# fuxiao0719/PanopticNeRF

Measured on AMD Instinct MI355X. Metric: Msamples/sec (coarse+fine), KITTI-360 1408x376, higher is better.
Workload: dtype bf16

## Files before the change

include/pnr.h:

```cpp
#ifndef PNR_H
#define PNR_H
#include <stdint.h>

#ifdef __cplusplus
extern "C" {
#endif

#define PNR_OK 0
#define PNR_EINVAL (-1)
#define PNR_EHIP (-2)
#define PNR_ENODEV (-3)

#define PNR_PREC_BF16 0
#define PNR_PREC_FP32 1

int pnr_version(void);
const char* pnr_last_error(void);
int pnr_device_check(int dev, char* buf_host, int buflen);

int pnr_stratified(const float* rays, int64_t n_rays, int n_samples, int lindisp,
                   const float* t_rand, float* z_out, void* stream);

int pnr_points(const float* rays, const float* z, int64_t n_rays, int n_samples, float* pts_out,
               void* stream);
// ... 3 lines not shown
typedef struct pnr_mlp_desc {
    int32_t D, W, skip;
    int32_t xyz_L, dir_L;
    int32_t n_sem, n_inst, head_W;
    int32_t precision;
    int32_t plan;
    int32_t head_tap;
    int32_t head_depth;
    int32_t schedule;
    int32_t clk_probe[2];
    int32_t flags;
} pnr_mlp_desc;

#define PNR_MLP_SOFTMAX 1
#define PNR_MLP_WG_CAP(n) (((n) & 0x1FF) << 16)
#define PNR_MLP_TRACE 0x7A00

typedef struct pnr_mlp_params_host {
    const float* const* pts_w; const float* const* pts_b;
    const float* alpha_w; const float* alpha_b;
    const float* feature_w; const float* feature_b;
    const float* views_w; const float* views_b;
    const float* rgb_w; const float* rgb_b;
    const float* sem0_w; const float* sem0_b; const float* sem1_w; const float* sem1_b;
    const float* inst0_w; const float* inst0_b; const float* inst1_w; const float* inst1_b;
} pnr_mlp_params_host;

int64_t pnr_mlp_packed_bytes(const pnr_mlp_desc* desc);
int pnr_mlp_pack(const pnr_mlp_desc* desc, const pnr_mlp_params_host* params, void* packed_host);

// ... 7 lines not shown
                    int64_t n_rays, int n_samples, float* raw, int64_t raw_stride_s,
                    int64_t raw_stride_c, void* stream);

int pnr_mlp_fused_plan(const pnr_mlp_desc* desc);
int64_t pnr_mlp_forward_composite_workspace_bytes(const pnr_mlp_desc* desc, int64_t n_rays, int n_samples, int want_weights);
int pnr_mlp_forward_composite(const pnr_mlp_desc* desc, const void* packed, const float* rays, const float* z,
                              int64_t n_rays, int n_samples, const int32_t* label_sem, const int32_t* label_inst,
                              int white_bkgd, float* rgb, float* depth, float* acc, float* weights, float* sem,
                              float* inst, float* fix_sem, float* fix_inst, void* workspace, void* stream);

int pnr_mlp_forward_tiles(const pnr_mlp_desc* desc, const void* packed, const float* rays, const float* z, int64_t n_rays,
                          int n_samples, void* workspace, void* stream);
int pnr_composite_combine(const pnr_mlp_desc* desc, const void* workspace, const float* z, int64_t n_rays, int n_samples,
                          const int32_t* label_sem, const int32_t* label_inst, int white_bkgd, float* rgb, float* depth,
                          float* acc, float* weights, float* sem, float* inst, float* fix_sem, float* fix_inst, void* stream);

int pnr_mlp_query(const pnr_mlp_desc* desc, const void* packed, const float* points, int64_t n_points,
                  float* sigma, int32_t* sem_label, int32_t* inst_label, int32_t* panoptic, const int32_t* is_thing,
                  float* sem_logits, float* inst_logits, int64_t logit_stride, void* stream);
int pnr_mlp_query_supported(const pnr_mlp_desc* desc);

int pnr_mlp_train_layout(const pnr_mlp_desc* desc, int64_t n_samples, int64_t* acts_off_host ,
                         int64_t* dys_off_host );
int pnr_mlp_forward_train(const pnr_mlp_desc* desc, const void* packed, const float* rays, const float* z,
                          int64_t n_rays, int n_samples, float* raw, int64_t raw_stride_s,
                          int64_t raw_stride_c, void* acts, void* stream);
int64_t pnr_mlp_bwd_packed_bytes(const pnr_mlp_desc* desc);
int pnr_mlp_pack_bwd(const pnr_mlp_desc* desc, const pnr_mlp_params_host* params, void* packed_host);
int pnr_mlp_backward(const pnr_mlp_desc* desc, const void* packed_bwd, const float* d_raw, const void* acts,
                     void* dys, int64_t n_rays, int n_samples, void* stream);
// ... 144 lines not shown
```

panopticnerf_amd/_lib.py:

```python
import ctypes
import os

_HERE = os.path.dirname(os.path.abspath(__file__))
LIB_PATH = os.environ.get("PNR_LIB_PATH") or os.path.join(_HERE, "libpnr.so")

c_f = ctypes.c_void_p
c_i64 = ctypes.c_int64
c_int = ctypes.c_int

PREC_BF16, PREC_FP32 = 0, 1
MLP_SOFTMAX, MLP_TRACE = 1, 0x7A00
CAMERA_PINHOLE, CAMERA_FISHEYE = 0, 1
TAG_PIXEL, TAG_FRAME = 16, 17
SAMPLE_POOLED, SAMPLE_FRAME = 0, 1


class LossCfg(ctypes.Structure):
    _fields_ = [("w_rgb", ctypes.c_float), ("w_depth", ctypes.c_float), ("w_sem", ctypes.c_float),
                ("w_fix_sem", ctypes.c_float), ("w_inst", ctypes.c_float), ("w_fix_inst", ctypes.c_float),
                ("depth_l2", ctypes.c_int32), ("fix_eps", ctypes.c_float), ("maps_are_prob", ctypes.c_int32)]


class MlpDesc(ctypes.Structure):
    _fields_ = [("D", ctypes.c_int32), ("W", ctypes.c_int32), ("skip", ctypes.c_int32),
                ("xyz_L", ctypes.c_int32), ("dir_L", ctypes.c_int32),
                ("n_sem", ctypes.c_int32), ("n_inst", ctypes.c_int32), ("head_W", ctypes.c_int32),
# ... 69 lines not shown
    "pnr_gen_rays": (c_int, [ctypes.POINTER(ctypes.c_float), ctypes.POINTER(ctypes.c_float), c_int, c_int, ctypes.c_float,
                             ctypes.c_float, c_f, c_i64, c_f, c_f]),
    "pnr_gen_rays_fisheye": (c_int, [ctypes.POINTER(ctypes.c_float), ctypes.POINTER(ctypes.c_float), c_int, c_int, ctypes.c_float,
                                     ctypes.c_float, c_f, c_i64, c_f, c_f, c_f]),
    "pnr_project_points": (c_int, [c_int, ctypes.POINTER(ctypes.c_float), ctypes.POINTER(ctypes.c_float), c_int, c_int, c_f, c_i64,
                                   c_f, c_f, c_f, c_f]),
    "pnr_panoptic_labels": (c_int, [c_f, c_f, c_f, c_i64, c_int, c_int, c_f, c_f, c_f, c_f]),
    "pnr_confusion": (c_int, [c_f, c_f, c_i64, c_int, c_f, c_f]),
    "pnr_sample_pdf": (c_int, [c_f, c_f, c_f, c_i64, c_int, c_int, c_f, c_f, c_f, c_f]),
    "pnr_bbox_hits": (c_int, [c_f, c_i64, c_f, c_int, c_int, c_f, c_f, c_f, c_f]),
    "pnr_restrict_rays": (c_int, [c_f, c_i64, c_f, c_f, c_int, c_f, c_f]),
    "pnr_sample_labels": (c_int, [c_f, c_i64, c_int, c_f, c_f, c_f, c_int, c_f, c_f, c_f, c_f]),
    "pnr_ray_setup": (c_int, [c_f, c_i64, c_f, c_int, c_int, c_f, c_int, c_int, c_f, c_int, c_f, c_f, c_f, c_f, c_f, c_f, c_f]),
    "pnr_sample_pdf_labels": (c_int, [c_f, c_f, c_f, c_i64, c_int, c_int, c_f, c_f, c_f, c_f, c_int, c_f, c_f, c_f, c_f]),
    "pnr_mlp_forward_tiles": (c_int, [ctypes.POINTER(MlpDesc), c_f, c_f, c_f, c_i64, c_int, c_f, c_f]),
    "pnr_rng_begin": (c_int, [c_f, c_f, c_f]),
    "pnr_rng_fill": (c_int, [ctypes.POINTER(RngDesc), c_i64, c_int, c_int, c_f, c_f]),
    "pnr_stratified_rng": (c_int, [c_f, c_i64, c_int, c_int, ctypes.POINTER(RngDesc), c_f, c_f]),
    "pnr_ray_setup_rng": (c_int, [c_f, c_i64, c_f, c_int, c_int, c_f, c_int, c_int, ctypes.POINTER(RngDesc), c_int, c_f, c_f, c_f, c_f,
                                  c_f, c_f, c_f]),
    "pnr_sample_pdf_rng": (c_int, [c_f, c_f, ctypes.POINTER(RngDesc), c_i64, c_int, c_int, c_f, c_f, c_f, c_f]),
    "pnr_sample_pdf_labels_rng": (c_int, [c_f, c_f, ctypes.POINTER(RngDesc), c_i64, c_int, c_int, c_f, c_f, c_f, c_f, c_int, c_f, c_f, c_f,
                                          c_f]),
    "pnr_composite_rng": (c_int, [c_f, c_i64, c_i64, c_f, c_f, ctypes.POINTER(RngDesc), c_f, c_f, c_i64, c_int, c_int, c_int, c_int,
                                  c_int, c_f, c_f, c_f, c_f, c_f, c_f, c_f, c_f, c_f]),
    "pnr_composite_backward_rng": (c_int, [c_f, c_i64, c_f, c_f, ctypes.POINTER(RngDesc), c_i64, c_int, c_int, c_int, c_int,
                                           c_f, c_f, c_f, c_f, c_f, c_f, c_f, c_f, c_f, c_f, c_f, c_f, c_f, c_f]),
    "pnr_sample_batch": (c_int, [c_f, c_f, c_f, c_int, ctypes.POINTER(RngDesc), c_i64, c_f, c_f, c_f, c_f, c_f, c_f, c_f, c_f]),
    "pnr_mlp_query": (c_int, [ctypes.POINTER(MlpDesc), c_f, c_f, c_i64, c_f, c_f, c_f, c_f, c_f, c_f, c_f, c_i64, c_f]),
    "pnr_mlp_query_supported": (c_int, [ctypes.POINTER(MlpDesc)]),
# ... 30 lines not shown
```

panopticnerf_amd/csrc/pnr_mlp.hip:

```cpp
#include <stdlib.h>
#include <string.h>

#include "pnr_mlp_plan.h"

int pnr_mlp_validate(const pnr_mlp_desc* d);

#include "pnr_mlp_core.h"
#include "pnr_mlp_pp.h"
#ifndef PNR_FUSE_TRANSPOSED
#define PNR_FUSE_TRANSPOSED 1
#endif
#include "pnr_mlp_fuse.h"
#include "pnr_mlp_tt.h"
#define PNR_QUERY_MAX_POINTS (((int64_t)1 << 31) - 4096)
#ifndef PNR_TRAIN_TILES_EXPERIMENT
#define PNR_TRAIN_TILES_EXPERIMENT 0
#endif
template <int PREC, int TILES, class CTX, int KIND, int NA, int NB, int NFB_OUT, int MODE, int NOUT>
__device__ __forceinline__ void layer_regs(CTX& c, const uint32_t (&inA)[TILES][NA],
                                           const uint32_t (&inB)[TILES][NB > 0 ? NB : 1],
                                           uint32_t (&out)[TILES][NOUT], uint16_t* save = nullptr,
                                           const int* srow = nullptr)
{
    constexpr int RPB = PrecT<PREC>::RPB;
// ... 818 lines not shown
{
    const int64_t i = (int64_t)blockIdx.x * 256 + threadIdx.x;
    if (i >= 2 * R) return;
    const int64_t ray = i >> 1;
    const int hi = (int)(i & 1);
    const float dx = rays[ray * 8 + 3], dy = rays[ray * 8 + 4], dz = rays[ray * 8 + 5];
    const float nrm = sqrtf(__fadd_rn(__fadd_rn(__fmul_rn(dx, dx), __fmul_rn(dy, dy)), __fmul_rn(dz, dz)));
    uint32_t ed[8];
    embed_lane<PNR_PREC_BF16, 2, 16, 8>(dx / nrm, dy / nrm, dz / nrm, hi, ed);
    uint4* o = reinterpret_cast<uint4*>(aux + i * 16);
    o[0] = make_uint4(ed[0], ed[1], ed[2], ed[3]);
    o[1] = make_uint4(ed[4], ed[5], ed[6], ed[7]);
    o[2] = make_uint4(__float_as_uint(nrm), 0u, 0u, 0u);
}

static int fused_mlp_launch(const pnr_mlp_desc* desc, const void* packed, const float* rays, const float* z, int64_t n_rays,
                            int n_samples, void* workspace, void* stream, MlpArgs& a)
{
    int rc = pnr_mlp_validate(desc);
    if (rc != PNR_OK) return rc;
    PNR_REQUIRE(desc->precision == PNR_PREC_BF16, "pnr_mlp_forward_composite: bf16 only");
    PNR_REQUIRE(desc->plan != 4, "pnr_mlp_forward_composite: a plan-4 (field) image is for pnr_mlp_query only");
    PNR_REQUIRE(n_rays >= 1 && n_samples >= 32 && n_samples <= 256 && (n_samples & 31) == 0,
                "pnr_mlp_forward_composite: n_samples=%d must be a multiple of 32 in [32,256]", n_samples);
    PNR_REQUIRE(desc->n_sem + desc->n_inst <= 128, "pnr_mlp_forward_composite: n_sem + n_inst <= 128");
    PNR_REQUIRE(packed && rays && z && workspace, "pnr_mlp_forward_composite: null pointer");
    PNR_REQUIRE(n_rays * (int64_t)n_samples < ((int64_t)1 << 31) - 4096, "pnr_mlp_forward_composite: R*N exceeds 2^31");
    PNR_REQUIRE((((uintptr_t)rays | (uintptr_t)packed | (uintptr_t)workspace) & 15) == 0,
                "pnr_mlp_forward_composite: rays / packed / workspace must be 16-byte aligned");
    PnrPlan plan;
// ... 3 lines not shown
    pnr_set_div_magic(n_samples, a.n_magic, a.n_shift);
    a.rec_floats = record_floats(*desc);
    a.rec = (float*)workspace;
    const int64_t tiles = ((int64_t)a.S + 255) / 256 * 8;
    a.ps = (float4*)(a.rec + tiles * a.rec_floats);
    hipStream_t st = (hipStream_t)stream;
    const bool softmax = (desc->flags & PNR_MLP_SOFTMAX) && desc->n_sem + desc->n_inst > 0;
    if (desc->plan == 3)
        return desc->W == 256 ? launch_mlp_pp<256, false, true, 0, true>(a, st) : launch_mlp_pp<128, false, true, 0, true>(a, st);
    if (desc->plan == 2) {
        PnrTTArgs t;
        memset(&t, 0, sizeof(t));
        t.image = a.data; t.rays = rays; t.z = z; t.S = a.S; t.N = a.N; t.n_magic = a.n_magic; t.n_shift = a.n_shift;
        t.rec = a.rec; t.rec_floats = a.rec_floats; t.ps = a.ps; t.n_sem = a.n_sem; t.n_inst = a.n_inst; t.clk = a.clk;
        PNR_REQUIRE(n_rays < ((int64_t)1 << 24), "pnr_mlp_forward_composite: the two-tile kernel addresses 2^24 rays per launch");
        uint32_t* aux = (uint32_t*)(((uintptr_t)((uint8_t*)a.ps + (int64_t)a.S * 16 + 256) + PNR_RAY_AUX_BYTES - 1)
                                    & ~(uintptr_t)(PNR_RAY_AUX_BYTES - 1));
        k_ray_aux<<<dim3((unsigned)((2 * n_rays + 255) / 256)), dim3(256), 0, st>>>(rays, n_rays, aux);
        t.aux = aux;
        t.n_wg = (desc->flags >> 16) & 0x1FF;
        if (pnr_tt_save_proto()) t.save = (void*)(((uintptr_t)((uint8_t*)aux + n_rays * PNR_RAY_AUX_BYTES) + 4095) & ~(uintptr_t)4095);
        const bool trace = (desc->flags & 0xFF00) == PNR_MLP_TRACE;
        return pnr_mlp_tt_launch(t, (desc->n_sem + 31) / 32, (desc->n_inst + 31) / 32, a.head_depth, a.head_tap, softmax, st, trace,
                                 trace ? ((desc->flags >> 4) & 7) : 0);
    }
    if (desc->plan == 1) {
        const int nbs = (desc->n_sem + 31) / 32, nbi = (desc->n_inst + 31) / 32;
        switch (4 * nbs + nbi + (softmax ? 16 : 0)) {
        case 4: return launch_mlp_pp<256, false, true, 4>(a, st);
        case 5: return launch_mlp_pp<256, false, true, 5>(a, st);
        case 8: return launch_mlp_pp<256, false, true, 8>(a, st);
        case 9: return launch_mlp_pp<256, false, true, 9>(a, st);
        case 20: return launch_mlp_pp<256, false, true, 20>(a, st);
// ... 258 lines not shown
```

panopticnerf_amd/csrc/pnr_mlp_pack.cpp:

```cpp
#include <math.h>
#include <string.h>

#include <vector>

#include "pnr_common.h"
#include "pnr_mlp_layout.h"
#include "pnr_mlp_plan.h"
#include "pnr_mlp_tt.h"

int pnr_mlp_validate(const pnr_mlp_desc* d)
{
    PNR_REQUIRE(d, "pnr_mlp: null desc");
    PNR_REQUIRE(d->W == 256 || d->W == 128, "pnr_mlp: W=%d unsupported (128 or 256)", d->W);
    PNR_REQUIRE(d->D >= 2 && d->D <= 16, "pnr_mlp: D=%d outside [2,16]", d->D);
    PNR_REQUIRE(d->skip >= -1 && d->skip < d->D - 1, "pnr_mlp: skip=%d must be -1 or < D-1", d->skip);
    PNR_REQUIRE(d->xyz_L >= 0 && d->xyz_L <= 10, "pnr_mlp: xyz_L=%d outside [0,10]", d->xyz_L);
    PNR_REQUIRE(d->dir_L >= 0 && d->dir_L <= 4, "pnr_mlp: dir_L=%d outside [0,4]", d->dir_L);
    PNR_REQUIRE(d->n_sem >= 0 && d->n_sem <= 256 && d->n_inst >= 0 && d->n_inst <= 256,
                "pnr_mlp: n_sem/n_inst outside [0,256]");
    PNR_REQUIRE((d->n_sem == 0 && d->n_inst == 0) || d->head_W == d->W / 2,
                "pnr_mlp: head_W=%d must equal W/2=%d", d->head_W, d->W / 2);
    PNR_REQUIRE(d->precision == PNR_PREC_BF16 || d->precision == PNR_PREC_FP32, "pnr_mlp: bad precision %d",
                d->precision);
    PNR_REQUIRE(d->head_tap == 0 || d->head_tap == 1, "pnr_mlp: head_tap=%d must be 0 (trunk output) or 1 (feature)", d->head_tap);
    PNR_REQUIRE(d->head_depth >= 0 && d->head_depth <= 2, "pnr_mlp: head_depth=%d must be 1 or 2", d->head_depth);
#ifndef PNR_TRAIN_TILES_EXPERIMENT
#define PNR_TRAIN_TILES_EXPERIMENT 0
#endif
    PNR_REQUIRE(d->schedule >= 0 && d->schedule <= (PNR_TRAIN_TILES_EXPERIMENT ? 6 : 2), "pnr_mlp: schedule=%d must be 0 (default), 1 (lock-step) or 2 (ping-pong)", d->schedule);
    PNR_REQUIRE(d->plan == 0 || (d->plan == 1 && pnr_plan1_supported(*d)) || (d->plan == 2 && pnr_plan2_supported(*d)) ||
                (d->plan == 3 && pnr_plan3_supported(*d)) || (d->plan == 4 && pnr_plan4_supported(*d)),
                "pnr_mlp: plan=%d is not available for this geometry (ask pnr_mlp_fused_plan; plans 3 and 4: bf16 only)", d->plan);
    const uint32_t trace = (uint32_t)d->flags & 0xFF00u;
    PNR_REQUIRE(((uint32_t)d->flags & ~(uint32_t)(PNR_MLP_SOFTMAX | 0xFF70u | PNR_MLP_WG_CAP(0x1FF))) == 0 && (trace == 0 || trace == PNR_MLP_TRACE) &&
                (trace != 0 || ((uint32_t)d->flags & 0x70u) == 0),
                "pnr_mlp: unknown bits in flags=0x%x (zero-initialise pnr_mlp_desc; PNR_MLP_* are the defined bits)", (unsigned)d->flags);
    PNR_REQUIRE(((uint32_t)d->clk_probe[0] & 15u) == 0, "pnr_mlp: clk_probe=0x%08x%08x is not a 16-byte aligned device address "
                "(zero-initialise pnr_mlp_desc; clk_probe is a diagnostics field, 0 = off)", (unsigned)d->clk_probe[1], (unsigned)d->clk_probe[0]);
    PNR_REQUIRE(trace == 0 || (d->clk_probe[0] | d->clk_probe[1]) != 0, "pnr_mlp: PNR_MLP_TRACE needs clk_probe");
    return PNR_OK;
}

PNR_EXPORT int pnr_mlp_fused_plan(const pnr_mlp_desc* desc)
{
    if (!desc) return 0;
    pnr_mlp_desc d = *desc;
    d.plan = 0;
    if (pnr_mlp_validate(&d) != PNR_OK) return 0;
    if ((d.flags & PNR_MLP_SOFTMAX) && d.n_sem + d.n_inst > 0)
// ... 341 lines not shown
```

panopticnerf_amd/csrc/pnr_sampling.hip:

```cpp
#include "pnr_camera_dev.h"
#include "pnr_common.h"
#include "pnr_philox.h"
#include <stdlib.h>
#include <string.h>

#pragma clang fp contract(off)

__device__ __forceinline__ float pnr_linspace01(int i, int N)
{
    if (N <= 1) return 0.0f;
    const float step = 1.0f / (float)(N - 1);
    if (i < N / 2) return step * (float)i;
    return fmaf(-step, (float)(N - 1 - i), 1.0f);
}

__device__ __forceinline__ float strat_z(float nr, float fr, int i, int N, int lindisp)
{
    const float t = pnr_linspace01(i, N);
    const float omt = 1.0f - t;
    if (!lindisp) {
        const float a = nr * omt, b = fr * t;
        return a + b;
    }
    const float a = (1.0f / nr) * omt, b = (1.0f / fr) * t;
// ... 288 lines not shown
        }
    }
}

#ifndef PDF_DET_WPE
#define PDF_DET_WPE 8
#endif
#if PDF_DET_WPE
__attribute__((amdgpu_waves_per_eu(PDF_DET_WPE, PDF_DET_WPE)))
#endif
__global__ __launch_bounds__(64) void k_sample_pdf_det(const float* __restrict__ z, const float* __restrict__ weights, int64_t R, int Nc,
                                                        int Nf, float* __restrict__ zfine_out, const PdfLabelArgs lab)
{
    __shared__ float s_z[64], s_w[64], s_pdf[64], s_cdf[64], s_bins[64];
    __shared__ float s_zs[192], s_out[256];
    __shared__ float s_total, s_part[32];
    const int lane = threadIdx.x;
    const int nb = Nc - 1, nw = Nc - 2, Nt = Nc + Nf;
    int topc = 1, topf = 1;
    while (topc * 2 <= Nc) topc *= 2;
    while (topf * 2 <= Nf) topf *= 2;
    const int mh = lab.max_hits;
    for (int64_t r = blockIdx.x; r < R; r += gridDim.x) {
        const float* __restrict__ zr = z + r * Nc;
        const float* __restrict__ wr = weights + r * Nc;
        const float zl = lane < Nc ? zr[lane] : 0.0f, wl = lane < Nc ? wr[lane] : 0.0f;
        int cnt = 0, h_ls = -1, h_li = -1;
        float h_ti = 0.0f, h_to = 0.0f;
        if (lab.label_sem) {
            const int c0 = lab.hit_count[r];
            cnt = c0 < mh ? c0 : mh;
            if (lane < cnt) {
                const float2 t2 = *reinterpret_cast<const float2*>(lab.hit_t + (r * mh + lane) * 2);
                h_ti = t2.x; h_to = t2.y;
                const int m = lab.hit_box[r * mh + lane];
                h_ls = lab.box_ids[m * 2];
                h_li = lab.box_ids[m * 2 + 1];
            }
        }
        s_z[lane] = zl;
        s_w[lane] = wl;
        const float zn = __shfl_down(zl, 1, 64), wn = __shfl_down(wl, 1, 64);
        s_bins[lane] = 0.5f * (zn + zl);
        __syncthreads();
        if (lane < 32) {
            const int k = lane >> 3, l = lane & 7, nv = nw / 8, groups = nv / 4;
            float pacc = 0.0f;
            for (int g = 0; g < groups; ++g) pacc = pacc + (s_w[(g * 4 + k) * 8 + l + 1] + 1e-5f);
            if (k == 0)
                for (int v = groups * 4; v < nv; ++v) pacc = pacc + (s_w[v * 8 + l + 1] + 1e-5f);
            s_part[lane] = pacc;
        }
        __syncthreads();
        if (lane == 0) {
            const int nv = nw / 8;
            float total = 0.0f;
            for (int j = nv * 8; j < nw; ++j) total = total + (s_w[j + 1] + 1e-5f);
            for (int l = 0; l < 8; ++l) {
                float p0 = s_part[l];
                p0 = p0 + s_part[8 + l]; p0 = p0 + s_part[16 + l]; p0 = p0 + s_part[24 + l];
                total = total + p0;
            }
            s_total = total;
        }
        __syncthreads();
        const float total = s_total;
        const float pl = lane < nw ? (wn + 1e-5f) / total : 0.0f;
        s_pdf[lane] = pl;
        double c = (double)pl;
        bool exact = __all(pl == 0.0f || pl >= 0x1p-28f);
        if (exact) {
#pragma unroll
            for (int d = 1; d < 64; d <<= 1) {
                const double o = __shfl_up(c, d, 64);
                if (lane >= d) c += o;
            }
            exact = __shfl(c, 63, 64) < 1.999;
        }
        if (exact) {
            if (lane == 0) s_cdf[0] = 0.0f;
            if (lane < nw) s_cdf[lane + 1] = (float)c;
// ... 18 lines not shown
                pos = (p <= nb && s_cdf[q - 1] <= uu) ? p : pos;
            }
            const int inds = pos;
            const int below = inds - 1 > 0 ? inds - 1 : 0;
            const int above = inds < nb - 1 ? inds : nb - 1;
            const float cb = s_cdf[below];
            float denom = s_cdf[above] - cb;
            if (denom < 1e-5f) denom = 1.0f;
            const float t = (uu - cb) / denom;
            const float bb = s_bins[below];
            const float span = s_bins[above] - bb;
            const float m = t * span;
            const float zs = bb + m;
            s_zs[i] = zs;
        }
        __syncthreads();
        for (int i = lane; i + 1 < Nf; i += 64) asc = asc && (s_zs[i] <= s_zs[i + 1]);
        if (__all(asc)) {
            if (lane < Nc) {
                int pos = 0;
                for (int st = topf; st >= 1; st >>= 1) {
                    const int p = pos + st, q = p <= Nf ? p : Nf;
                    pos = (p <= Nf && s_zs[q - 1] < zl) ? p : pos;
                }
                s_out[lane + pos] = zl;
            }
            for (int j = lane; j < Nf; j += 64) {
                const float v = s_zs[j];
                int pos = 0;
                for (int st = topc; st >= 1; st >>= 1) {
                    const int p = pos + st, q = p <= Nc ? p : Nc;
                    pos = (p <= Nc && s_z[q - 1] <= v) ? p : pos;
                }
                s_out[j + pos] = v;
            }
            __syncthreads();
        } else {
            int P = 1;
            while (P < Nt) P <<= 1;
            pdf_bitonic_fallback(s_out, s_z, s_zs, Nc, Nf, P, lane);
        }
        float* __restrict__ zo = zfine_out + r * Nt;
        for (int i0 = 0; i0 < Nt; i0 += 256) {
            float zz[4];
            int best[4], ls[4], li[4];
            float bt[4];
#pragma unroll
            for (int k = 0; k < 4; ++k) {
                const int i = i0 + lane + 64 * k;
                zz[k] = i < Nt ? s_out[i < Nt ? i : 0] : 0.0f;
                best[k] = -1; ls[k] = -1; li[k] = -1; bt[k] = 0.0f;
                if (i < Nt) zo[i] = zz[k];
            }
            if (lab.label_sem) {
                for (int h = 0; h < cnt; ++h) {
                    const float ti = __int_as_float(__builtin_amdgcn_readlane(__float_as_int(h_ti), h));
                    const float to = __int_as_float(__builtin_amdgcn_readlane(__float_as_int(h_to), h));
                    const int hs = __builtin_amdgcn_readlane(h_ls, h), hi2 = __builtin_amdgcn_readlane(h_li, h);
#pragma unroll
                    for (int k = 0; k < 4; ++k) {
                        const bool take = ti <= zz[k] && zz[k] <= to && (best[k] < 0 || ti < bt[k]);
                        best[k] = take ? h : best[k];
                        bt[k] = take ? ti : bt[k];
                        ls[k] = take ? hs : ls[k];
                        li[k] = take ? hi2 : li[k];
                    }
                }
#pragma unroll
                for (int k = 0; k < 4; ++k) {
                    const int i = i0 + lane + 64 * k;
                    if (i < Nt) {
                        lab.label_sem[r * Nt + i] = ls[k];
                        lab.label_inst[r * Nt + i] = li[k];
                    }
                }
            }
        }
        __syncthreads();
    }
}

__global__ __launch_bounds__(64) __attribute__((amdgpu_waves_per_eu(8, 8)))
void k_sample_pdf(const float* __restrict__ z, const float* __restrict__ weights, const float* __restrict__ u, int64_t R, int Nc, int Nf,
                  float* __restrict__ zs_out, int32_t* __restrict__ inds_out, float* __restrict__ zfine_out, const PdfLabelArgs lab)
{
    sample_pdf_body<64, 256>(z, weights, u, R, Nc, Nf, zs_out, inds_out, zfine_out, lab);
}
__global__ __launch_bounds__(64)
void k_sample_pdf_big(const float* __restrict__ z, const float* __restrict__ weights, const float* __restrict__ u, int64_t R, int Nc, int Nf,
                      float* __restrict__ zs_out, int32_t* __restrict__ inds_out, float* __restrict__ zfine_out, const PdfLabelArgs lab)
{
    sample_pdf_body<PDF_MAXC, PDF_MAXT>(z, weights, u, R, Nc, Nf, zs_out, inds_out, zfine_out, lab);
// ... 510 lines not shown
```

panopticnerf_amd/ops.py:

```python
import ctypes
import os

import torch

from . import _lib
from ._lib import MlpDesc, MlpParamsHost


def _stream():
    return ctypes.c_void_p(torch.cuda.current_stream().cuda_stream)


def _chk(t, name, dtype=torch.float32):
    if t is None:
        return None
    if not t.is_cuda:
        raise RuntimeError(f"{name}: expected a GPU tensor (the HIP path has no CPU fallback)")
    if t.dtype != dtype:
        raise TypeError(f"{name}: expected {dtype}, got {t.dtype}")
    if not t.is_contiguous():
        raise ValueError(f"{name}: tensor must be contiguous")
    return t


# ... 494 lines not shown
        ok = int(_lib.load().pnr_mlp_fused_plan(ctypes.byref(desc_for_mode(desc, 1)))) >= 1
    return ok


def desc_for_mode(desc, sem_mode):
    want = _lib.MLP_SOFTMAX if int(sem_mode) == 1 else 0
    if (desc.flags & _lib.MLP_SOFTMAX) == want:
        return desc
    return _desc_with(desc, flags=(desc.flags & ~_lib.MLP_SOFTMAX) | want)


def fused_image(sem_mode=0):
    return "softmax" if int(sem_mode) == 1 else True


@_on_device
def mlp_forward_composite(desc, packed, rays, z, label_sem=None, label_inst=None, white_bkgd=False, want_weights=True, out=None,
                          sem_mode=0, wg_cap=0):
    rays, z, packed = _chk(rays, "rays"), _chk(z, "z"), _chk(packed, "packed", torch.uint8)
    label_sem = _chk(label_sem, "label_sem", torch.int32)
    label_inst = _chk(label_inst, "label_inst", torch.int32)
    R, N = z.shape
    n_sem, n_inst = desc.n_sem, desc.n_inst
    dev = z.device
    lib = _lib.load()
    desc = desc_for_mode(desc, sem_mode)
    if wg_cap:
        desc = _desc_with(desc, flags=(desc.flags & 0xFFFF) | ((int(wg_cap) & 0x1FF) << 16))
    nbytes = lib.pnr_mlp_forward_composite_workspace_bytes(ctypes.byref(desc), R, N, int(bool(want_weights)))
    if nbytes < 0:
        raise RuntimeError("pnr_mlp_forward_composite: unsupported geometry (n_samples=%d must be a multiple of 32)" % N)
    ws = torch.empty(int(nbytes), device=dev, dtype=torch.uint8)
    out = _maps(out, R, N, n_sem, n_inst, label_sem, label_inst, want_weights, dev)
    g = out.get
    _lib.check(lib.pnr_mlp_forward_composite(ctypes.byref(desc), _p(packed), _p(rays), _p(z), R, N, _p(label_sem), _p(label_inst),
                                             int(bool(white_bkgd)), _p(out["rgb"]), _p(out["depth"]), _p(out["acc"]),
                                             _p(g("weights")), _p(g("semantic")), _p(g("instance")), _p(g("fix_semantic")),
                                             _p(g("fix_instance")), _p(ws), _stream()), "pnr_mlp_forward_composite")
    return out


WEIGHTS_ONLY_DROPS = ("rgb", "semantic", "instance")


def sigma_pass_supported(desc, n_samples, noise=None):
    if not (desc.precision == _lib.PREC_BF16 and noise is None and n_samples % 32 == 0 and 32 <= n_samples <= 256
            and desc.n_sem + desc.n_inst <= 128):
# ... 293 lines not shown
```

panopticnerf_amd/renderer.py:

```python
import os

import torch

from . import ops


def _get(cfg, name, default):
    return getattr(cfg, name, default) if cfg is not None else default


CHUNK_QUANTUM = 1024


PREAMBLE_EARLY = os.environ.get("PNR_OVERLAP_PRE", "1") != "0"
CHUNK_TAIL = 8


def chunk_plan(n_rays, chunk_size):
    n_rays, chunk_size = int(n_rays), max(1, int(chunk_size))
    if n_rays <= 0:
        return []
    n = -(-n_rays // chunk_size)
    if n > 1 and n_rays - (n - 1) * chunk_size <= chunk_size // CHUNK_TAIL:
        n -= 1
# ... 53 lines not shown
                             "cfg.share_coarse_fine = True to evaluate one NeRF at both levels on purpose" % self.N_importance)

    def _preamble(self, rays, box, box_ids, t_rand, z_out):
        hits = lab0 = None
        hull = self.bbox_sampling == "hull"
        if box is not None and self.max_hits <= ops.RAY_SETUP_MAX_HITS:
            hits, z, ls0, li0 = ops.ray_setup(rays, box, box_ids, self.N_samples, self.max_hits, self.lindisp, t_rand, hull, out=z_out)
            lab0 = (ls0, li0)
        else:
            if box is not None:
                hits = ops.bbox_hits(rays, box, self.max_hits)
            rays_s = ops.restrict_rays(rays, hits[0], hits[2]) if (hits is not None and hull) else rays
            z = ops.stratified(rays_s, self.N_samples, self.lindisp, t_rand, out=z_out)
        return hits, z, lab0

    def render_rays(self, rays, box=None, box_ids=None, t_rand=None, u=None, train=False, grad=False, out=None, sched=None, rng=None):
        net, Nc, Nf = self.net, self.N_samples, self.N_importance
        n0 = net.nerf(0)
        C, K = n0.n_sem, n0.n_inst
        dev = rays.device
        ret = {}
        hits = lab0 = None
        if t_rand is None and self.perturb > 0 and train:
            t_rand = ops.Draw(rng[0], 1, rng[1]) if rng is not None else torch.rand((rays.shape[0], Nc), device=dev)
        own = (lambda key: out.get(key)) if (out and not grad) else (lambda key: None)
        if sched is not None and sched.get("pre") is not None:
            hits, z, lab0 = sched["pre"]
        else:
            hits, z, lab0 = self._preamble(rays, box, box_ids, t_rand, own("z_vals_0"))
        if hits is not None and self.strict_hits:
            over = torch.stack([(hits[2] > self.max_hits).sum(), hits[2].max()])
            self._overflow = over if self._overflow is None else torch.stack([self._overflow[0] + over[0],
                                                                              torch.maximum(self._overflow[1], over[1])])

        def level(lv, zz, labels=None):
            ls = li = None
            if labels is not None:
                ls, li = labels
            elif hits is not None:
                ls, li = ops.sample_labels(zz, hits[0], hits[1], hits[2], box_ids)
            noise = None
            if self.raw_noise_std > 0 and train:
                if rng is not None:
                    noise = ops.Draw(rng[0], 3 + lv, rng[1], self.raw_noise_std)
# ... 10 lines not shown
                    res = ops.mlp_forward_weights(desc, img, rays, zz, ls, li, out=mine)
                else:
                    desc, img = net.packed(0, dev)
                    raw = ops.mlp_forward(desc, img, rays, zz, channel_major=True)
                    res = ops.composite(raw, zz, rays, C, K, True, noise, ls, li, self.sem_mode, self.white_bkgd, True, out=mine)
                    res = {k: v for k, v in res.items() if k not in ops.WEIGHTS_ONLY_DROPS}
            else:
                need_w = self.keep_weights or (lv == 0 and Nf > 0)
                mine = {k: own(f"{k}_{lv}") for k in ("rgb", "depth", "acc", "weights", "semantic", "instance", "fix_semantic", "fix_instance")}
                mine = {k: v for k, v in mine.items() if v is not None}
                if self.fuse and ops.fused_supported(net.nerf(lv).desc(net.precision), zz.shape[1], self.sem_mode, noise):
                    desc, img = net.packed(lv, dev, fused=ops.fused_image(self.sem_mode))
                    if sched is not None and lv == 0 and sched.get("wait") is not None:
                        torch.cuda.current_stream(dev).wait_event(sched["wait"])
                    res = ops.mlp_forward_composite(desc, img, rays, zz, ls, li, self.white_bkgd, need_w, out=mine, sem_mode=self.sem_mode,
                                                    wg_cap=0 if sched is None else sched["caps"][lv])
                else:
                    desc, img = net.packed(lv, dev)
                    raw = ops.mlp_forward(desc, img, rays, zz, channel_major=True)
                    res = ops.composite(raw, zz, rays, C, K, True, noise, ls, li, self.sem_mode, self.white_bkgd, need_w, out=mine)
            for k, v in res.items():
                ret[f"{k}_{lv}"] = v
            ret[f"z_vals_{lv}"] = zz
            return res

        o0 = level(0, z, lab0)
        if Nf > 0:
            if u is None and self.perturb > 0 and train:
                u = ops.Draw(rng[0], 2, rng[1]) if rng is not None else torch.rand((rays.shape[0], Nf), device=dev)
            w0 = o0["weights"].detach().contiguous()
            if hits is not None:
                z_fine, ls1, li1 = ops.sample_pdf_labels(z, w0, Nf, hits, box_ids, u, out=own("z_vals_1"))
                lab1 = (ls1, li1)
            else:
                z_fine, _, _ = ops.sample_pdf(z, w0, Nf, u, want_samples=False, out=own("z_vals_1"))
                lab1 = None
            if sched is not None:
                sched["pdf_done"] = torch.cuda.Event()
                sched["pdf_done"].record(torch.cuda.current_stream(dev))
                if sched.get("before_fine") is not None:
                    sched["before_fine"]()
            level(1, z_fine, lab1)
        return ret

    def _empty_outputs(self, lead, has_box, dev, grad=False):
        n0 = self.net.nerf(0)
        C, K = n0.n_sem, n0.n_inst
        ret = {}
        for lv, N in ((0, self.N_samples),) + (((1, self.N_samples + self.N_importance),) if self.N_importance > 0 else ()):
            need_w = self.keep_weights or (lv == 0 and self.N_importance > 0)
            drop = ops.WEIGHTS_ONLY_DROPS if (lv == 0 and not grad and self.coarse_outputs == "weights") else ()
            m = ops._maps(None, 0, N, C, K, True if has_box else None, True if has_box else None, need_w, dev, drop=drop)
            m["z_vals"] = torch.empty((0, N), device=dev, dtype=torch.float32)
            for k, v in m.items():
                ret[f"{k}_{lv}"] = v.reshape(*lead, *v.shape[1:])
        return ret

# ... 28 lines not shown

    def _render_overlapped(self, rays, box, box_ids, plan, caps, lead):
        dev = rays.device
        R = rays.shape[0]
        cap_c, cap_f = caps
        frame = self._frame_maps(R, box is not None, dev)
        main = torch.cuda.current_stream(dev)
        if dev not in self._side_streams:
            self._side_streams[dev] = (torch.cuda.Stream(dev), torch.cuda.Stream(dev))
        side = self._side_streams[dev]
        start = torch.cuda.Event()
        start.record(main)
        for st in side:
            st.wait_event(start)
        prev_pdf = None
        pre = {}

        def preamble(cj):
            sj, ej = plan[cj]
            pre[cj] = self._preamble(rays[sj:ej], box, box_ids, None, frame["z_vals_0"][sj:ej])
        for ci, (s, e) in enumerate(plan):
            sched = {"wait": prev_pdf, "caps": (0 if ci == 0 else cap_c, 0 if ci == len(plan) - 1 else cap_f), "pdf_done": None,
                     "pre": pre.pop(ci, None),
                     "before_fine": (lambda cj=ci + 2: preamble(cj)) if (PREAMBLE_EARLY and ci + 2 < len(plan)) else None}
            with torch.cuda.stream(side[ci & 1]):
                o = self.render_rays(rays[s:e], box, box_ids, None, None, False, False, out={k: v[s:e] for k, v in frame.items()}, sched=sched)
                for k, v in o.items():
                    if v.data_ptr() != frame[k][s:e].data_ptr():
                        frame[k][s:e].copy_(v)
            prev_pdf = sched["pdf_done"]
        for st in side:
            done = torch.cuda.Event()
            done.record(st)
            main.wait_event(done)
        return {k: v.reshape(*lead, *v.shape[1:]) for k, v in frame.items()}

    def render(self, batch):
        rays = batch["rays"]
        if not rays.is_cuda:
            raise RuntimeError("Renderer.render: batch['rays'] must be on the GPU (no CPU fallback)")
        grad = torch.is_grad_enabled() and any(p.requires_grad for p in self.net.parameters())
# ... 20 lines not shown
        caps = self._overlap_caps(rays.device, plan, grad, train, box is not None, t_rand, u)
        if caps is not None:
            return self._render_overlapped(rays, box, box_ids, plan, caps, lead)
        call = None
        if self.rng == "device" and train and (self.perturb > 0 or self.raw_noise_std > 0):
            if self.rng_state.device != rays.device:
                self.rng_state = self.rng_state.to(rays.device)
            call = ops.rng_begin(self.rng_state)
        outs = []
        frame = None
        for s, e in plan:
            o = self.render_rays(rays[s:e], box, box_ids,
                                 None if t_rand is None else t_rand[s:e],
                                 None if u is None else u[s:e], train, grad,
                                 out=None if frame is None else {k: v[s:e] for k, v in frame.items()},
                                 rng=None if call is None else (call, s))
            if s == 0 and e < R and not grad and self.frame_outputs and all(v.dim() >= 1 and v.shape[0] == e for v in o.values()):
                frame = {k: torch.empty((R,) + tuple(v.shape[1:]), device=v.device, dtype=v.dtype) for k, v in o.items()}
                for k, v in o.items():
                    frame[k][:e].copy_(v)
            elif frame is not None:
                for k, v in o.items():
                    if v.data_ptr() != frame[k][s:e].data_ptr():
                        frame[k][s:e].copy_(v)
            outs.append(o)
        if self._overflow is not None:
            n_over, worst = (int(v) for v in self._overflow.tolist())
            self._overflow = None
            if n_over > 0:
                raise RuntimeError("Renderer.render: %d ray(s) cross more than max_hits = %d boxes (up to %d): the farthest "
                                   "intervals were dropped -- raise cfg.max_hits" % (n_over, self.max_hits, worst))
# ... 49 lines not shown
```

Measured before the change: 1150.

## Prefill per-ray aux tables ahead of fused launches and software-pipeline PDF sampling

Adds a standalone pnr_ray_aux entry point and an AUX_READY flag so the per-ray aux table for the two-tile fused kernel can be built ahead of time into a caller-owned workspace. In the overlapped renderer this is scheduled two chunks ahead after the fine pass, which takes the small kernel off the critical path. Separately, the PDF-sampling kernel now prefetches the next ray's z, weights and hit data while working on the current ray, and does the weight-sum reduction with readlane instead of shared memory and two barriers. The cost is extra workspace allocations per chunk, more live registers, and more scheduling complexity.

```diff
diff --git a/include/pnr.h b/include/pnr.h
--- a/include/pnr.h
+++ b/include/pnr.h
@@ -41,6 +41,7 @@
 
 #define PNR_MLP_SOFTMAX 1
 #define PNR_MLP_WG_CAP(n) (((n) & 0x1FF) << 16)
+#define PNR_MLP_AUX_READY 4
 #define PNR_MLP_TRACE 0x7A00
 
 typedef struct pnr_mlp_params_host {
@@ -78,6 +79,8 @@
 int pnr_composite_combine(const pnr_mlp_desc* desc, const void* workspace, const float* z, int64_t n_rays, int n_samples,
                           const int32_t* label_sem, const int32_t* label_inst, int white_bkgd, float* rgb, float* depth,
                           float* acc, float* weights, float* sem, float* inst, float* fix_sem, float* fix_inst, void* stream);
+
+int pnr_ray_aux(const pnr_mlp_desc* desc, const float* rays, int64_t n_rays, int n_samples, void* workspace, void* stream);
 
 int pnr_mlp_query(const pnr_mlp_desc* desc, const void* packed, const float* points, int64_t n_points,
                   float* sigma, int32_t* sem_label, int32_t* inst_label, int32_t* panoptic, const int32_t* is_thing,
diff --git a/panopticnerf_amd/_lib.py b/panopticnerf_amd/_lib.py
--- a/panopticnerf_amd/_lib.py
+++ b/panopticnerf_amd/_lib.py
@@ -9,7 +9,7 @@
 c_int = ctypes.c_int
 
 PREC_BF16, PREC_FP32 = 0, 1
-MLP_SOFTMAX, MLP_TRACE = 1, 0x7A00
+MLP_SOFTMAX, MLP_AUX_READY, MLP_TRACE = 1, 4, 0x7A00
 CAMERA_PINHOLE, CAMERA_FISHEYE = 0, 1
 TAG_PIXEL, TAG_FRAME = 16, 17
 SAMPLE_POOLED, SAMPLE_FRAME = 0, 1
@@ -109,6 +109,7 @@
     "pnr_ray_setup": (c_int, [c_f, c_i64, c_f, c_int, c_int, c_f, c_int, c_int, c_f, c_int, c_f, c_f, c_f, c_f, c_f, c_f, c_f]),
     "pnr_sample_pdf_labels": (c_int, [c_f, c_f, c_f, c_i64, c_int, c_int, c_f, c_f, c_f, c_f, c_int, c_f, c_f, c_f, c_f]),
     "pnr_mlp_forward_tiles": (c_int, [ctypes.POINTER(MlpDesc), c_f, c_f, c_f, c_i64, c_int, c_f, c_f]),
+    "pnr_ray_aux": (c_int, [ctypes.POINTER(MlpDesc), c_f, c_i64, c_int, c_f, c_f]),
     "pnr_rng_begin": (c_int, [c_f, c_f, c_f]),
     "pnr_rng_fill": (c_int, [ctypes.POINTER(RngDesc), c_i64, c_int, c_int, c_f, c_f]),
     "pnr_stratified_rng": (c_int, [c_f, c_i64, c_int, c_int, ctypes.POINTER(RngDesc), c_f, c_f]),
diff --git a/panopticnerf_amd/csrc/pnr_mlp.hip b/panopticnerf_amd/csrc/pnr_mlp.hip
--- a/panopticnerf_amd/csrc/pnr_mlp.hip
+++ b/panopticnerf_amd/csrc/pnr_mlp.hip
@@ -856,6 +856,34 @@
     o[2] = make_uint4(__float_as_uint(nrm), 0u, 0u, 0u);
 }
 
+static uint32_t* ray_aux_region(const pnr_mlp_desc& desc, void* workspace, int64_t n_rays, int n_samples)
+{
+    const int64_t S = n_rays * n_samples, tiles = (S + 255) / 256 * 8;
+    uint8_t* ps = (uint8_t*)((float*)workspace + tiles * record_floats(desc));
+    return (uint32_t*)(((uintptr_t)(ps + S * 16 + 256) + PNR_RAY_AUX_BYTES - 1) & ~(uintptr_t)(PNR_RAY_AUX_BYTES - 1));
+}
+
+static void ray_aux_launch(const float* rays, int64_t n_rays, uint32_t* aux, hipStream_t st)
+{
+    k_ray_aux<<<dim3((unsigned)((2 * n_rays + 255) / 256)), dim3(256), 0, st>>>(rays, n_rays, aux);
+}
+
+PNR_EXPORT int pnr_ray_aux(const pnr_mlp_desc* desc, const float* rays, int64_t n_rays, int n_samples, void* workspace, void* stream)
+{
+    int rc = pnr_mlp_validate(desc);
+    if (rc != PNR_OK) return rc;
+    PNR_REQUIRE(desc->plan == 2, "pnr_ray_aux: only the plan-2 (two-tile) launch reads a per-ray table, not plan %d", desc->plan);
+    PNR_REQUIRE(n_rays >= 0 && n_samples >= 32 && n_samples <= 256 && (n_samples & 31) == 0,
+                "pnr_ray_aux: n_samples=%d must be a multiple of 32 in [32,256]", n_samples);
+    if (n_rays == 0) return PNR_OK;
+    PNR_REQUIRE(rays && workspace, "pnr_ray_aux: null pointer");
+    PNR_REQUIRE(n_rays < ((int64_t)1 << 24) && n_rays * (int64_t)n_samples < ((int64_t)1 << 31) - 4096, "pnr_ray_aux: too many rays");
+    PNR_REQUIRE((((uintptr_t)rays | (uintptr_t)workspace) & 15) == 0, "pnr_ray_aux: rays / workspace must be 16-byte aligned");
+    ray_aux_launch(rays, n_rays, ray_aux_region(*desc, workspace, n_rays, n_samples), (hipStream_t)stream);
+    PNR_CHECK_LAUNCH("pnr_ray_aux");
+    return PNR_OK;
+}
+
 static int fused_mlp_launch(const pnr_mlp_desc* desc, const void* packed, const float* rays, const float* z, int64_t n_rays,
                             int n_samples, void* workspace, void* stream, MlpArgs& a)
 {
@@ -889,9 +917,8 @@
         t.image = a.data; t.rays = rays; t.z = z; t.S = a.S; t.N = a.N; t.n_magic = a.n_magic; t.n_shift = a.n_shift;
         t.rec = a.rec; t.rec_floats = a.rec_floats; t.ps = a.ps; t.n_sem = a.n_sem; t.n_inst = a.n_inst; t.clk = a.clk;
         PNR_REQUIRE(n_rays < ((int64_t)1 << 24), "pnr_mlp_forward_composite: the two-tile kernel addresses 2^24 rays per launch");
-        uint32_t* aux = (uint32_t*)(((uintptr_t)((uint8_t*)a.ps + (int64_t)a.S * 16 + 256) + PNR_RAY_AUX_BYTES - 1)
-                                    & ~(uintptr_t)(PNR_RAY_AUX_BYTES - 1));
-        k_ray_aux<<<dim3((unsigned)((2 * n_rays + 255) / 256)), dim3(256), 0, st>>>(rays, n_rays, aux);
+        uint32_t* aux = ray_aux_region(*desc, workspace, n_rays, n_samples);
+        if (!(desc->flags & PNR_MLP_AUX_READY)) ray_aux_launch(rays, n_rays, aux, st);
         t.aux = aux;
         t.n_wg = (desc->flags >> 16) & 0x1FF;
         if (pnr_tt_save_proto()) t.save = (void*)(((uintptr_t)((uint8_t*)aux + n_rays * PNR_RAY_AUX_BYTES) + 4095) & ~(uintptr_t)4095);
diff --git a/panopticnerf_amd/csrc/pnr_mlp_pack.cpp b/panopticnerf_amd/csrc/pnr_mlp_pack.cpp
--- a/panopticnerf_amd/csrc/pnr_mlp_pack.cpp
+++ b/panopticnerf_amd/csrc/pnr_mlp_pack.cpp
@@ -32,7 +32,7 @@
                 (d->plan == 3 && pnr_plan3_supported(*d)) || (d->plan == 4 && pnr_plan4_supported(*d)),
                 "pnr_mlp: plan=%d is not available for this geometry (ask pnr_mlp_fused_plan; plans 3 and 4: bf16 only)", d->plan);
     const uint32_t trace = (uint32_t)d->flags & 0xFF00u;
-    PNR_REQUIRE(((uint32_t)d->flags & ~(uint32_t)(PNR_MLP_SOFTMAX | 0xFF70u | PNR_MLP_WG_CAP(0x1FF))) == 0 && (trace == 0 || trace == PNR_MLP_TRACE) &&
+    PNR_REQUIRE(((uint32_t)d->flags & ~(uint32_t)(PNR_MLP_SOFTMAX | PNR_MLP_AUX_READY | 0xFF70u | PNR_MLP_WG_CAP(0x1FF))) == 0 && (trace == 0 || trace == PNR_MLP_TRACE) &&
                 (trace != 0 || ((uint32_t)d->flags & 0x70u) == 0),
                 "pnr_mlp: unknown bits in flags=0x%x (zero-initialise pnr_mlp_desc; PNR_MLP_* are the defined bits)", (unsigned)d->flags);
     PNR_REQUIRE(((uint32_t)d->clk_probe[0] & 15u) == 0, "pnr_mlp: clk_probe=0x%08x%08x is not a 16-byte aligned device address "
diff --git a/panopticnerf_amd/csrc/pnr_sampling.hip b/panopticnerf_amd/csrc/pnr_sampling.hip
--- a/panopticnerf_amd/csrc/pnr_sampling.hip
+++ b/panopticnerf_amd/csrc/pnr_sampling.hip
@@ -326,28 +326,44 @@
 {
     __shared__ float s_z[64], s_w[64], s_pdf[64], s_cdf[64], s_bins[64];
     __shared__ float s_zs[192], s_out[256];
-    __shared__ float s_total, s_part[32];
     const int lane = threadIdx.x;
     const int nb = Nc - 1, nw = Nc - 2, Nt = Nc + Nf;
     int topc = 1, topf = 1;
     while (topc * 2 <= Nc) topc *= 2;
     while (topf * 2 <= Nf) topf *= 2;
     const int mh = lab.max_hits;
-    for (int64_t r = blockIdx.x; r < R; r += gridDim.x) {
-        const float* __restrict__ zr = z + r * Nc;
-        const float* __restrict__ wr = weights + r * Nc;
-        const float zl = lane < Nc ? zr[lane] : 0.0f, wl = lane < Nc ? wr[lane] : 0.0f;
-        int cnt = 0, h_ls = -1, h_li = -1;
-        float h_ti = 0.0f, h_to = 0.0f;
-        if (lab.label_sem) {
-            const int c0 = lab.hit_count[r];
-            cnt = c0 < mh ? c0 : mh;
-            if (lane < cnt) {
-                const float2 t2 = *reinterpret_cast<const float2*>(lab.hit_t + (r * mh + lane) * 2);
-                h_ti = t2.x; h_to = t2.y;
-                const int m = lab.hit_box[r * mh + lane];
-                h_ls = lab.box_ids[m * 2];
-                h_li = lab.box_ids[m * 2 + 1];
+    const bool has_lab = lab.label_sem != nullptr;
+    int64_t r = blockIdx.x;
+    if (r >= R) return;
+    float zl = lane < Nc ? z[r * Nc + lane] : 0.0f, wl = lane < Nc ? weights[r * Nc + lane] : 0.0f;
+    int cnt = 0, h_ls = -1, h_li = -1;
+    float h_ti = 0.0f, h_to = 0.0f;
+    if (has_lab) {
+        const int c0 = lab.hit_count[r];
+        cnt = c0 < mh ? c0 : mh;
+        if (lane < cnt) {
+            const float2 t2 = *reinterpret_cast<const float2*>(lab.hit_t + (r * mh + lane) * 2);
+            h_ti = t2.x; h_to = t2.y;
+            const int m = lab.hit_box[r * mh + lane];
+            h_ls = lab.box_ids[m * 2];
+            h_li = lab.box_ids[m * 2 + 1];
+        }
+    }
+    asm volatile("" : "+v"(zl), "+v"(wl), "+v"(h_ti), "+v"(h_to), "+v"(h_ls), "+v"(h_li));
+    for (;;) {
+        const int64_t rn = r + gridDim.x;
+        const bool more = rn < R;
+        float n_zl = 0.0f, n_wl = 0.0f;
+        int n_c0 = 0, n_box = -1;
+        float2 n_t = make_float2(0.0f, 0.0f);
+        if (more) {
+            if (lane < Nc) { n_zl = z[rn * Nc + lane]; n_wl = weights[rn * Nc + lane]; }
+            if (has_lab) {
+                if (lane == 0) n_c0 = lab.hit_count[rn];
+                if (lane < mh) {
+                    n_t = *reinterpret_cast<const float2*>(lab.hit_t + (rn * mh + lane) * 2);
+                    n_box = lab.hit_box[rn * mh + lane];
+                }
             }
         }
         s_z[lane] = zl;
@@ -355,28 +371,24 @@
         const float zn = __shfl_down(zl, 1, 64), wn = __shfl_down(wl, 1, 64);
         s_bins[lane] = 0.5f * (zn + zl);
         __syncthreads();
+        float pacc = 0.0f;
         if (lane < 32) {
             const int k = lane >> 3, l = lane & 7, nv = nw / 8, groups = nv / 4;
-            float pacc = 0.0f;
             for (int g = 0; g < groups; ++g) pacc = pacc + (s_w[(g * 4 + k) * 8 + l + 1] + 1e-5f);
             if (k == 0)
                 for (int v = groups * 4; v < nv; ++v) pacc = pacc + (s_w[v * 8 + l + 1] + 1e-5f);
-            s_part[lane] = pacc;
-        }
-        __syncthreads();
-        if (lane == 0) {
-            const int nv = nw / 8;
-            float total = 0.0f;
-            for (int j = nv * 8; j < nw; ++j) total = total + (s_w[j + 1] + 1e-5f);
-            for (int l = 0; l < 8; ++l) {
-                float p0 = s_part[l];
-                p0 = p0 + s_part[8 + l]; p0 = p0 + s_part[16 + l]; p0 = p0 + s_part[24 + l];
-                total = total + p0;
-            }
-            s_total = total;
-        }
-        __syncthreads();
-        const float total = s_total;
+        }
+        float total = 0.0f;
+        for (int j = (nw / 8) * 8; j < nw; ++j)
+            total = total + (__int_as_float(__builtin_amdgcn_readlane(__float_as_int(wl), j + 1)) + 1e-5f);
+#pragma unroll
+        for (int l = 0; l < 8; ++l) {
+            float p0 = __int_as_float(__builtin_amdgcn_readlane(__float_as_int(pacc), l));
+            p0 = p0 + __int_as_float(__builtin_amdgcn_readlane(__float_as_int(pacc), 8 + l));
+            p0 = p0 + __int_as_float(__builtin_amdgcn_readlane(__float_as_int(pacc), 16 + l));
+            p0 = p0 + __int_as_float(__builtin_amdgcn_readlane(__float_as_int(pacc), 24 + l));
+            total = total + p0;
+        }
         const float pl = lane < nw ? (wn + 1e-5f) / total : 0.0f;
         s_pdf[lane] = pl;
         double c = (double)pl;
@@ -425,6 +437,16 @@
             const float zs = bb + m;
             s_zs[i] = zs;
         }
+        asm volatile("" : "+v"(n_zl), "+v"(n_wl), "+v"(n_c0), "+v"(n_box), "+v"(n_t.x), "+v"(n_t.y));
+        int n_cnt = 0, n_ls = -1, n_li = -1;
+        if (more && has_lab) {
+            const int c0 = __builtin_amdgcn_readfirstlane(n_c0);
+            n_cnt = c0 < mh ? c0 : mh;
+            if (lane < n_cnt) {
+                n_ls = lab.box_ids[n_box * 2];
+                n_li = lab.box_ids[n_box * 2 + 1];
+            }
+        }
         __syncthreads();
         for (int i = lane; i + 1 < Nf; i += 64) asc = asc && (s_zs[i] <= s_zs[i + 1]);
         if (__all(asc)) {
@@ -451,42 +473,52 @@
             while (P < Nt) P <<= 1;
             pdf_bitonic_fallback(s_out, s_z, s_zs, Nc, Nf, P, lane);
         }
+        float zz[4];
+        int ls[4], li[4];
+#pragma unroll
+        for (int k = 0; k < 4; ++k) {
+            const int i = lane + 64 * k;
+            zz[k] = i < Nt ? s_out[i < Nt ? i : 0] : 0.0f;
+            ls[k] = -1; li[k] = -1;
+        }
+        if (has_lab) {
+            int best[4];
+            float bt[4];
+#pragma unroll
+            for (int k = 0; k < 4; ++k) { best[k] = -1; bt[k] = 0.0f; }
+            for (int h = 0; h < cnt; ++h) {
+                const float ti = __int_as_float(__builtin_amdgcn_readlane(__float_as_int(h_ti), h));
+                const float to = __int_as_float(__builtin_amdgcn_readlane(__float_as_int(h_to), h));
+                const int hs = __builtin_amdgcn_readlane(h_ls, h), hi2 = __builtin_amdgcn_readlane(h_li, h);
+#pragma unroll
+                for (int k = 0; k < 4; ++k) {
+                    const bool take = ti <= zz[k] && zz[k] <= to && (best[k] < 0 || ti < bt[k]);
+                    best[k] = take ? h : best[k];
+                    bt[k] = take ? ti : bt[k];
+                    ls[k] = take ? hs : ls[k];
+                    li[k] = take ? hi2 : li[k];
+                }
+            }
+        }
+        asm volatile("" : "+v"(n_ls), "+v"(n_li));
         float* __restrict__ zo = zfine_out + r * Nt;
-        for (int i0 = 0; i0 < Nt; i0 += 256) {
-            float zz[4];
-            int best[4], ls[4], li[4];
-            float bt[4];
-#pragma unroll
-            for (int k = 0; k < 4; ++k) {
-                const int i = i0 + lane + 64 * k;
-                zz[k] = i < Nt ? s_out[i < Nt ? i : 0] : 0.0f;
-                best[k] = -1; ls[k] = -1; li[k] = -1; bt[k] = 0.0f;
-                if (i < Nt) zo[i] = zz[k];
-            }
-            if (lab.label_sem) {
-                for (int h = 0; h < cnt; ++h) {
-                    const float ti = __int_as_float(__builtin_amdgcn_readlane(__float_as_int(h_ti), h));
-                    const float to = __int_as_float(__builtin_amdgcn_readlane(__float_as_int(h_to), h));
-                    const int hs = __builtin_amdgcn_readlane(h_ls, h), hi2 = __builtin_amdgcn_readlane(h_li, h);
-#pragma unroll
-                    for (int k = 0; k < 4; ++k) {
-                        const bool take = ti <= zz[k] && zz[k] <= to && (best[k] < 0 || ti < bt[k]);
-                        best[k] = take ? h : best[k];
-                        bt[k] = take ? ti : bt[k];
-                        ls[k] = take ? hs : ls[k];
-                        li[k] = take ? hi2 : li[k];
-                    }
-                }
-#pragma unroll
-                for (int k = 0; k < 4; ++k) {
-                    const int i = i0 + lane + 64 * k;
-                    if (i < Nt) {
-                        lab.label_sem[r * Nt + i] = ls[k];
-                        lab.label_inst[r * Nt + i] = li[k];
-                    }
-                }
-            }
-        }
+#pragma unroll
+        for (int k = 0; k < 4; ++k) {
+            const int i = lane + 64 * k;
+            if (i < Nt) {
+                zo[i] = zz[k];
+                if (has_lab) {
+                    lab.label_sem[r * Nt + i] = ls[k];
+                    lab.label_inst[r * Nt + i] = li[k];
+                }
+            }
+        }
+        if (!more) break;
+        r = rn;
+        zl = n_zl; wl = n_wl;
+        cnt = n_cnt;
+        h_ti = n_t.x; h_to = n_t.y;
+        h_ls = n_ls; h_li = n_li;
         __syncthreads();
     }
 }
diff --git a/panopticnerf_amd/ops.py b/panopticnerf_amd/ops.py
--- a/panopticnerf_amd/ops.py
+++ b/panopticnerf_amd/ops.py
@@ -532,9 +532,36 @@
     return "softmax" if int(sem_mode) == 1 else True
 
 
+def _workspace_bytes(desc, R, N):
+    nbytes = _lib.load().pnr_mlp_forward_composite_workspace_bytes(ctypes.byref(desc), R, N, 1)
+    if nbytes < 0:
+        raise RuntimeError("pnr_mlp_forward_composite: unsupported geometry (n_samples=%d must be a multiple of 32)" % N)
+    return int(nbytes)
+
+
+def fused_workspace(desc, n_rays, n_samples, dev):
+    return torch.empty(_workspace_bytes(desc, int(n_rays), int(n_samples)), device=dev, dtype=torch.uint8)
+
+
+def _chk_workspace(ws, desc, R, N, dev):
+    if not (isinstance(ws, torch.Tensor) and ws.dtype == torch.uint8 and ws.device == dev and ws.is_contiguous()
+            and ws.numel() >= _workspace_bytes(desc, R, N)):
+        raise ValueError("workspace must be a contiguous uint8 tensor of fused_workspace(desc, %d, %d, %s)" % (R, N, dev))
+    return ws
+
+
+@_on_device
+def ray_aux(desc, rays, n_samples, workspace):
+    rays = _chk(rays, "rays")
+    R = rays.shape[0]
+    ws = _chk_workspace(workspace, desc, R, int(n_samples), rays.device)
+    _lib.check(_lib.load().pnr_ray_aux(ctypes.byref(desc), _p(rays), R, int(n_samples), _p(ws), _stream()), "pnr_ray_aux")
+    return ws
+
+
 @_on_device
 def mlp_forward_composite(desc, packed, rays, z, label_sem=None, label_inst=None, white_bkgd=False, want_weights=True, out=None,
-                          sem_mode=0, wg_cap=0):
+                          sem_mode=0, wg_cap=0, workspace=None, aux_ready=False):
     rays, z, packed = _chk(rays, "rays"), _chk(z, "z"), _chk(packed, "packed", torch.uint8)
     label_sem = _chk(label_sem, "label_sem", torch.int32)
     label_inst = _chk(label_inst, "label_inst", torch.int32)
@@ -545,10 +572,11 @@
     desc = desc_for_mode(desc, sem_mode)
     if wg_cap:
         desc = _desc_with(desc, flags=(desc.flags & 0xFFFF) | ((int(wg_cap) & 0x1FF) << 16))
-    nbytes = lib.pnr_mlp_forward_composite_workspace_bytes(ctypes.byref(desc), R, N, int(bool(want_weights)))
-    if nbytes < 0:
-        raise RuntimeError("pnr_mlp_forward_composite: unsupported geometry (n_samples=%d must be a multiple of 32)" % N)
-    ws = torch.empty(int(nbytes), device=dev, dtype=torch.uint8)
+    if aux_ready:
+        if workspace is None:
+            raise ValueError("mlp_forward_composite: aux_ready needs the workspace ray_aux() filled")
+        desc = _desc_with(desc, flags=desc.flags | _lib.MLP_AUX_READY)
+    ws = fused_workspace(desc, R, N, dev) if workspace is None else _chk_workspace(workspace, desc, R, N, dev)
     out = _maps(out, R, N, n_sem, n_inst, label_sem, label_inst, want_weights, dev)
     g = out.get
     _lib.check(lib.pnr_mlp_forward_composite(ctypes.byref(desc), _p(packed), _p(rays), _p(z), R, N, _p(label_sem), _p(label_inst),
diff --git a/panopticnerf_amd/renderer.py b/panopticnerf_amd/renderer.py
--- a/panopticnerf_amd/renderer.py
+++ b/panopticnerf_amd/renderer.py
@@ -91,7 +91,24 @@
             z = ops.stratified(rays_s, self.N_samples, self.lindisp, t_rand, out=z_out)
         return hits, z, lab0
 
-    def render_rays(self, rays, box=None, box_ids=None, t_rand=None, u=None, train=False, grad=False, out=None, sched=None, rng=None):
+    def _prefill_aux(self, rays):
+        ws = {}
+        if not self.fuse or os.environ.get("PNR_AUX_PREFILL", "1") == "0":
+            return ws
+        net, dev, R = self.net, rays.device, rays.shape[0]
+        levels = ((0, self.N_samples),) + (((1, self.N_samples + self.N_importance),) if self.N_importance > 0 else ())
+        for lv, N in levels:
+            if lv == 0 and self.coarse_outputs == "weights":
+                continue
+            if not ops.fused_supported(net.nerf(lv).desc(net.precision), N, self.sem_mode, None):
+                continue
+            desc, _ = net.packed(lv, dev, fused=ops.fused_image(self.sem_mode))
+            if desc.plan == 2:
+                ws[lv] = ops.ray_aux(desc, rays, N, ops.fused_workspace(desc, R, N, dev))
+        return ws
+
+    def render_rays(self, rays, box=None, box_ids=None, t_rand=None, u=None, train=False, grad=False, out=None, sched=None, rng=None,
+                    prefill=False):
         net, Nc, Nf = self.net, self.N_samples, self.N_importance
         n0 = net.nerf(0)
         C, K = n0.n_sem, n0.n_inst
@@ -105,6 +122,10 @@
             hits, z, lab0 = sched["pre"]
         else:
             hits, z, lab0 = self._preamble(rays, box, box_ids, t_rand, own("z_vals_0"))
+        if sched is not None and sched.get("aux") is not None:
+            aux = sched["aux"]
+        else:
+            aux = self._prefill_aux(rays) if (prefill and not grad and not (self.raw_noise_std > 0 and train)) else {}
         if hits is not None and self.strict_hits:
             over = torch.stack([(hits[2] > self.max_hits).sum(), hits[2].max()])
             self._overflow = over if self._overflow is None else torch.stack([self._overflow[0] + over[0],
@@ -145,7 +166,8 @@
                     if sched is not None and lv == 0 and sched.get("wait") is not None:
                         torch.cuda.current_stream(dev).wait_event(sched["wait"])
                     res = ops.mlp_forward_composite(desc, img, rays, zz, ls, li, self.white_bkgd, need_w, out=mine, sem_mode=self.sem_mode,
-                                                    wg_cap=0 if sched is None else sched["caps"][lv])
+                                                    wg_cap=0 if sched is None else sched["caps"][lv], workspace=aux.get(lv),
+                                                    aux_ready=lv in aux)
                 else:
                     desc, img = net.packed(lv, dev)
                     raw = ops.mlp_forward(desc, img, rays, zz, channel_major=True)
@@ -172,6 +194,8 @@
                 if sched.get("before_fine") is not None:
                     sched["before_fine"]()
             level(1, z_fine, lab1)
+            if sched is not None and sched.get("after_fine") is not None:
+                sched["after_fine"]()
         return ret
 
     def _empty_outputs(self, lead, has_box, dev, grad=False):
@@ -230,17 +254,23 @@
         for st in side:
             st.wait_event(start)
         prev_pdf = None
-        pre = {}
+        pre, aux = {}, {}
 
         def preamble(cj):
             sj, ej = plan[cj]
             pre[cj] = self._preamble(rays[sj:ej], box, box_ids, None, frame["z_vals_0"][sj:ej])
+
+        def tables(cj):
+            sj, ej = plan[cj]
+            aux[cj] = self._prefill_aux(rays[sj:ej])
         for ci, (s, e) in enumerate(plan):
             sched = {"wait": prev_pdf, "caps": (0 if ci == 0 else cap_c, 0 if ci == len(plan) - 1 else cap_f), "pdf_done": None,
-                     "pre": pre.pop(ci, None),
+                     "pre": pre.pop(ci, None), "aux": aux.pop(ci, None),
+                     "after_fine": (lambda cj=ci + 2: tables(cj)) if ci + 2 < len(plan) else None,
                      "before_fine": (lambda cj=ci + 2: preamble(cj)) if (PREAMBLE_EARLY and ci + 2 < len(plan)) else None}
             with torch.cuda.stream(side[ci & 1]):
-                o = self.render_rays(rays[s:e], box, box_ids, None, None, False, False, out={k: v[s:e] for k, v in frame.items()}, sched=sched)
+                o = self.render_rays(rays[s:e], box, box_ids, None, None, False, False, out={k: v[s:e] for k, v in frame.items()}, sched=sched,
+                                     prefill=True)
                 for k, v in o.items():
                     if v.data_ptr() != frame[k][s:e].data_ptr():
                         frame[k][s:e].copy_(v)
@@ -291,7 +321,7 @@
                                  None if t_rand is None else t_rand[s:e],
                                  None if u is None else u[s:e], train, grad,
                                  out=None if frame is None else {k: v[s:e] for k, v in frame.items()},
-                                 rng=None if call is None else (call, s))
+                                 rng=None if call is None else (call, s), prefill=not grad)
             if s == 0 and e < R and not grad and self.frame_outputs and all(v.dim() >= 1 and v.shape[0] == e for v in o.values()):
                 frame = {k: torch.empty((R,) + tuple(v.shape[1:]), device=v.device, dtype=v.dtype) for k, v in o.items()}
                 for k, v in o.items():
```

Result: no change. 1150, median of 4 (+0.0%).
